# kubernetes-sigs/lws

Hardware: AMD Instinct MI355X
Metric: replica-group time-to-ready + rollout p50; Llama-3-70B 1-leader/0-worker TP=1 (lower is better)
Workload: dtype bf16; 1 GPU; model=llama-3-70b, global_batch=32, seq_len=128, parallelism=tp1, group=1-leader/0-workers (size=1), replicas=1, collectives_staged=False, orchestrator=lws_amd in-process control plane

## Files before the change

### lws_amd/cluster/statefulset_controller.py

```python
from __future__ import annotations

import re
from typing import Optional

from ..api import serde
from ..api.core import ControllerRevision, Pod, StatefulSet
from ..api.meta import OwnerReference, get_int_or_percent
from ..utils.hashutil import hash_object
from .controller import Controller, Manager
from .store import AlreadyExistsError, NotFoundError, Store

POD_NAME_RE = re.compile(r"^(.*)-([0-9]+)$")
STS_REVISION_LABEL = "controller-revision-hash"
STS_POD_NAME_LABEL = "statefulset.kubernetes.io/pod-name"
STS_OWNER_LABEL = "lws.amd.com/statefulset-name"


def parse_parent_and_ordinal(name: str) -> tuple[Optional[str], int]:
    m = POD_NAME_RE.match(name)
    if not m:
        return None, -1
    return m.group(1), int(m.group(2))


# ... 120 lines not shown
        cr = self.store.try_get("ControllerRevision", sts.metadata.namespace, name)
        if cr is None:
            return serde.deep_copy(sts.spec.template)
        from ..api.core import PodTemplateSpec
        return serde.from_dict(PodTemplateSpec, cr.data["template"])

    def _create_pod(self, sts: StatefulSet, ordinal: int, rev: str) -> None:
        template = self._template_for_revision(sts, rev)
        pod = Pod(metadata=serde.deep_copy(template.metadata),
                  spec=serde.deep_copy(template.spec))
        pod.metadata.name = f"{sts.metadata.name}-{ordinal}"
        pod.metadata.namespace = sts.metadata.namespace
        pod.metadata.labels = dict(template.metadata.labels or {})
        pod.metadata.labels[STS_REVISION_LABEL] = rev
        pod.metadata.labels[STS_POD_NAME_LABEL] = pod.metadata.name
        pod.metadata.labels[STS_OWNER_LABEL] = sts.metadata.name
        pod.metadata.annotations = dict(template.metadata.annotations or {})
        pod.metadata.owner_references = [OwnerReference(
            api_version=sts.api_version, kind=sts.kind, name=sts.metadata.name,
            uid=sts.metadata.uid, controller=True, block_owner_deletion=True)]
        pod.spec.hostname = pod.metadata.name
        if not pod.spec.subdomain:
            pod.spec.subdomain = sts.spec.service_name
        try:
            self.store.create(pod)
        except AlreadyExistsError:
            return
        self._ensure_pvcs(sts, pod)

    def _ensure_pvcs(self, sts: StatefulSet, pod: Pod) -> None:
        from ..api import serde as _serde

        created = self.store.try_get("Pod", pod.metadata.namespace,
                                     pod.metadata.name)
        if created is None:
            return
        policy = sts.spec.persistent_volume_claim_retention_policy
        for vct in sts.spec.volume_claim_templates or []:
            pvc = _serde.deep_copy(vct)
            pvc.metadata.name = f"{vct.metadata.name}-{pod.metadata.name}"
            pvc.metadata.namespace = sts.metadata.namespace
            pvc.metadata.labels = dict(vct.metadata.labels or {})
            pvc.metadata.labels[STS_OWNER_LABEL] = sts.metadata.name
            pvc.metadata.owner_references = []
            if policy is not None and policy.when_scaled == "Delete":
                pvc.metadata.owner_references = [OwnerReference(
# ... 54 lines not shown
```

### lws_amd/controllers/leaderworkerset_controller.py

```python
from __future__ import annotations

from typing import Optional

from ..api import leaderworkerset as lwsapi
from ..api import serde
from ..api.core import (RollingUpdateStatefulSetStrategy, Service,
                        ServiceSpec, StatefulSet, StatefulSetSpec,
                        StatefulSetUpdateStrategy)
from ..api.leaderworkerset import LeaderWorkerSet
from ..api.meta import (LabelSelector, OwnerReference, format_label_selector,
                        get_int_or_percent, new_condition)
from ..cluster.controller import Controller, Manager
from ..cluster.statefulset_controller import statefulset_ready
from ..cluster.store import AlreadyExistsError, Store
from ..utils import revision as revisionutils
from ..utils.podutils import pod_running_and_ready

FIELD_MANAGER = "lws"


def _merge_metadata(base: dict[str, str], overrides: dict[str, str]) -> dict[str, str]:
    out = dict(base or {})
    out.update(overrides)
    return out
# ... 333 lines not shown
             lwsapi.REVISION_KEY: revision_key})
        sts.metadata.annotations = _merge_metadata(
            lws.metadata.annotations,
            {lwsapi.REPLICAS_ANNOTATION_KEY: str(lws.spec.replicas)})
        sts.metadata.owner_references = [OwnerReference(
            api_version=lws.api_version, kind=lws.kind, name=lws.metadata.name,
            uid=lws.metadata.uid, controller=True, block_owner_deletion=True)]
        sts.spec = StatefulSetSpec(
            replicas=replicas,
            service_name=lws.metadata.name,
            pod_management_policy="Parallel",
            template=template,
            update_strategy=StatefulSetUpdateStrategy(
                type=lws.spec.rollout_strategy.type,
                rolling_update=RollingUpdateStatefulSetStrategy(
                    partition=partition,
                    max_unavailable=sts_max_unavailable)),
            selector=LabelSelector(match_labels={
                lwsapi.SET_NAME_LABEL_KEY: lws.metadata.name,
                lwsapi.WORKER_INDEX_LABEL_KEY: "0"}),
            volume_claim_templates=serde.deep_copy(t.volume_claim_templates),
            persistent_volume_claim_retention_policy=serde.deep_copy(
                t.persistent_volume_claim_retention_policy))
        self.store.apply(sts, field_manager=FIELD_MANAGER)

    def _reconcile_headless_services(self, lws) -> None:
        if lws.spec.network_config is not None and \
                lws.spec.network_config.subdomain_policy == \
                lwsapi.SubdomainPolicy.UniquePerReplica:
            return
        if self.store.try_get("Service", lws.metadata.namespace,
                              lws.metadata.name) is not None:
            return
        svc = Service()
        svc.metadata.name = lws.metadata.name
        svc.metadata.namespace = lws.metadata.namespace
        svc.spec = ServiceSpec(
            cluster_ip="None",
            selector={lwsapi.SET_NAME_LABEL_KEY: lws.metadata.name},
            publish_not_ready_addresses=True)
        svc.metadata.owner_references = [OwnerReference(
            api_version=lws.api_version, kind=lws.kind, name=lws.metadata.name,
            uid=lws.metadata.uid, controller=True, block_owner_deletion=True)]
        try:
            self.store.create(svc)
        except AlreadyExistsError:
# ... 101 lines not shown
```

### lws_amd/models/llama.py

```python
from __future__ import annotations

import math
from dataclasses import dataclass
import torch

from ..parallel.tp import ShardedLinear, all_gather_cat, all_reduce


@dataclass
class LlamaConfig:
    name: str = "llama"
    hidden_size: int = 4096
    intermediate_size: int = 14336
    num_layers: int = 32
    num_q_heads: int = 32
    num_kv_heads: int = 8
    head_dim: int = 128
    vocab_size: int = 128256
    rope_theta: float = 500000.0
    rms_eps: float = 1e-5
    max_position: int = 8192
    num_experts: int = 0
    num_experts_per_tok: int = 2

# ... 164 lines not shown
        else:
            lins += [self.gate_up, self.down]
        for lin in lins:
            lin.materialize(gen)
        self.input_norm.fill_(1.0)
        self.post_norm.fill_(1.0)

    @property
    def param_count(self) -> int:
        n = self.qkv.numel + self.o.numel
        n += self.input_norm.numel() + self.post_norm.numel()
        if self.router is not None:
            n += self.router.numel()
            n += sum(l.numel for l in self.experts_gate_up)
            n += sum(l.numel for l in self.experts_down)
        else:
            n += self.gate_up.numel + self.down.numel
        return n


class LlamaForCausalLM:
    def __init__(self, cfg: LlamaConfig, tp_rank: int = 0, tp_world: int = 1,
                 device: str = "cpu", dtype=torch.bfloat16,
                 pp_rank: int = 0, pp_world: int = 1):
        self.cfg = cfg
        self.tp_rank = tp_rank
        self.tp_world = tp_world
        self.pp_rank = pp_rank
        self.pp_world = pp_world
        assert tp_world == 1 or pp_world == 1, \
            "combined TP x PP grids are not supported"
        self.device = torch.device(device)
        self.dtype = dtype
        self._ops = _Ops(self.device)
        L, base, rem = cfg.num_layers, cfg.num_layers // pp_world, \
            cfg.num_layers % pp_world
        sizes = [base + (1 if r < rem else 0) for r in range(pp_world)]
        self.layer_offset = sum(sizes[:pp_rank])
        self.pp_first = pp_rank == 0
        self.pp_last = pp_rank == pp_world - 1
        self.layers = [LlamaLayer(cfg, tp_rank, tp_world, self.device, dtype)
                       for _ in range(sizes[pp_rank])]
        self.embed = torch.empty(cfg.vocab_size, cfg.hidden_size,
                                 device=self.device, dtype=dtype) \
            if self.pp_first else None
        self.final_norm = torch.empty(cfg.hidden_size, device=self.device,
                                      dtype=dtype) if self.pp_last else None
        self.lm_head = ShardedLinear(cfg.vocab_size, cfg.hidden_size, 0,
# ... 86 lines not shown
            k_cache[s // page, :, s % page] = k[t]
            v_cache[s // page, :, s % page] = v[t]

    def _qkv_views(self, qkv: torch.Tensor, layer, positions):
        d = self.cfg.head_dim
        if self._ops.is_gpu:
            q = qkv.narrow(-1, 0, layer.q_slice).unflatten(-1, (layer.hq, d))
            k = qkv.narrow(-1, layer.q_slice,
                           layer.kv_slice).unflatten(-1, (layer.hkv, d))
            v = qkv.narrow(-1, layer.q_slice + layer.kv_slice,
                           layer.kv_slice).unflatten(-1, (layer.hkv, d))
            self._ops.ops.rope(q, k, self.rope_table, positions,
                               layer.hq, layer.hkv)
            return q, k, v
        q, k, v = qkv.split([layer.q_slice, layer.kv_slice, layer.kv_slice],
                            dim=-1)
        q, k = self._ops.ref.rope_ref(q.contiguous(), k.contiguous(),
                                      self.rope_table, positions,
                                      layer.hq, layer.hkv)
        T = qkv.size(0)
        return (q.view(T, layer.hq, d), k.view(T, layer.hkv, d),
                v.contiguous().view(T, layer.hkv, d))

    def forward_prefill(self, batch: PrefillBatch, kv_caches) -> torch.Tensor:
        cfg = self.cfg
        if self.pp_first:
            x = self.embed[batch.input_ids]
            residual = None
        else:
            from ..parallel import pp as ppmod
            T = batch.input_ids.size(0)
            st = ppmod.recv_stage((2, T, cfg.hidden_size), self.dtype,
                                  self.device, self.pp_rank - 1)
            x, residual = st[0], st[1]
        for li, layer in enumerate(self.layers):
            if residual is None:
                residual = x
                h = self._rmsnorm(x, layer.input_norm)
            else:
                h, residual = self._fused_add_rmsnorm(x, residual,
                                                      layer.input_norm)
            qkv = layer.qkv(h)
            q, k, v = self._qkv_views(qkv, layer, batch.positions)
            k_cache, v_cache = kv_caches[li]
            self._write_cache(k, v, k_cache, v_cache, batch.slot_mapping)
            attn = self._prefill_attention(q, k, v, batch, layer,
                                           k_cache, v_cache)
# ... 33 lines not shown
        out = torch.empty(T, layer.hq * d, device=q.device, dtype=q.dtype)
        G = layer.hq // layer.hkv
        offs = q_offsets or [0] * (len(batch.seq_starts) - 1)
        for i in range(len(batch.seq_starts) - 1):
            s0, s1 = batch.seq_starts[i], batch.seq_starts[i + 1]
            kv0, kv1 = kv_starts[i], kv_starts[i + 1]
            S, KV, off = s1 - s0, kv1 - kv0, offs[i]
            qs = q[s0:s1].transpose(0, 1)
            ks = k[kv0:kv1].transpose(0, 1)
            vs = v[kv0:kv1].transpose(0, 1)
            ks = ks.repeat_interleave(G, dim=0)
            vs = vs.repeat_interleave(G, dim=0)
            scores = (qs @ ks.transpose(-1, -2)).float() * self.scale
            cols = torch.arange(KV, device=q.device)
            rows = torch.arange(S, device=q.device)
            mask = torch.where(cols[None, :] > off + rows[:, None],
                               float("-inf"), 0.0)
            p = torch.softmax(scores + mask, dim=-1).to(q.dtype)
            o = (p @ vs).transpose(0, 1).reshape(S, layer.hq * d)
            out[s0:s1] = o
        return out

    def forward_decode(self, batch: DecodeBatch, kv_caches) -> torch.Tensor:
        cfg = self.cfg
        if self.pp_first:
            x = self.embed[batch.input_ids]
            residual = None
        else:
            from ..parallel import pp as ppmod
            B0 = batch.input_ids.size(0)
            st = ppmod.recv_stage((2, B0, cfg.hidden_size), self.dtype,
                                  self.device, self.pp_rank - 1)
            x, residual = st[0], st[1]
        fp8q = (self._ops.is_gpu and self.layers
                and getattr(self.layers[0].qkv, "weight_fp8", None)
                is not None and self.layers[0].router is None
                and x.size(0) <= 32 and cfg.hidden_size % 256 == 0
                and self.layers[0].down.weight_fp8.size(1) % 256 == 0)
        for li, layer in enumerate(self.layers):
            if fp8q:
                if residual is None:
                    residual = x
                    h8, hs = self._ops.ops.rmsnorm_fp8(x, layer.input_norm,
                                                       cfg.rms_eps)
                else:
                    h8, hs = self._ops.ops.fused_add_rmsnorm_fp8(
# ... 113 lines not shown
```

### lws_amd/ops/__init__.py

```python
from __future__ import annotations

from pathlib import Path
from typing import Optional

import torch

_LIB = None
_LOAD_ERROR: Optional[str] = None


def _try_load() -> None:
    global _LIB, _LOAD_ERROR
    if _LIB is not None or _LOAD_ERROR is not None:
        return
    so = Path(__file__).resolve().parent / "_C.so"
    if not so.exists():
        _LOAD_ERROR = f"{so} not built (run python -m lws_amd.ops.build)"
        return
    try:
        torch.ops.load_library(str(so))
    except Exception:
        pass
    try:
        import importlib.util
# ... 53 lines not shown
    lib.rope(q, k, cos_sin, positions, num_q_heads, num_kv_heads)


def rope_and_cache(q, k, v, cos_sin, positions, k_cache, v_cache,
                   slot_mapping) -> None:
    lib = require_native()
    lib.rope_and_cache(q, k, v, cos_sin, positions, k_cache, v_cache,
                       slot_mapping)


def build_rope_table(max_pos: int, head_dim: int, theta: float = 10000.0,
                     device="cpu") -> torch.Tensor:
    half = head_dim // 2
    inv_freq = 1.0 / (theta ** (torch.arange(0, half, dtype=torch.float64) / half))
    pos = torch.arange(max_pos, dtype=torch.float64)
    ang = torch.outer(pos, inv_freq)
    table = torch.cat([torch.cos(ang), torch.sin(ang)], dim=-1).float()
    return table.to(device)


_PA_WS: dict = {}


def paged_attention_decode(q: torch.Tensor, k_cache: torch.Tensor,
                           v_cache: torch.Tensor, block_tables: torch.Tensor,
                           seq_lens: torch.Tensor, scale: float,
                           chunk_keys: Optional[int] = None,
                           workspace: Optional[tuple] = None,
                           out: Optional[torch.Tensor] = None) -> torch.Tensor:
    import os as _os

    lib = require_native()
    B, Hq, D = q.shape
    Hkv = k_cache.size(1)
    G = Hq // Hkv
    mfma = G in (4, 8, 16) and _os.environ.get("LWS_PA_MFMA", "1") != "0"
    max_len = int(block_tables.size(1)) * int(k_cache.size(2))
    if chunk_keys is None:
        if B * Hkv >= 256 and G == 1 and max_len <= 512:
            chunk_keys = ((max_len + 15) // 16) * 16
        else:
            if B * Hkv <= 64:
                if mfma:
                    target_chunks = max(1, min(8, -(-max_len // 64)))
                else:
                    target_chunks = min(16, (max_len + 31) // 32)
            else:
                target_chunks = max(1, min(4, -(-max_len // 96)))
            chunk_keys = -(-max_len // target_chunks)
            chunk_keys = ((chunk_keys + 15) // 16) * 16
    num_chunks = max(1, (max_len + chunk_keys - 1) // chunk_keys)
    if mfma:
        num_chunks *= 4
    if workspace is None:
        key = ("paws", B, Hkv, num_chunks, G, q.device.index)
        ws = _PA_WS.get(key)
        if ws is None:
            ws = (torch.empty((B, Hkv, num_chunks, G, D),
                              dtype=torch.float32, device=q.device),
                  torch.empty((B, Hkv, num_chunks, G, 2),
                              dtype=torch.float32, device=q.device))
            _PA_WS[key] = ws
        ws_acc, ws_ml = ws
    else:
        ws_acc, ws_ml = workspace
        num_chunks = ws_ml.size(2)
    if out is None:
        out = torch.empty_like(q)
    lib.paged_attention_decode(out, q, k_cache, v_cache, block_tables,
                               seq_lens, ws_acc, ws_ml, scale, chunk_keys)
    return out


def reshape_and_cache(k: torch.Tensor, v: torch.Tensor, k_cache: torch.Tensor,
                      v_cache: torch.Tensor, slot_mapping: torch.Tensor) -> None:
    lib = require_native()
    lib.reshape_and_cache(k, v, k_cache, v_cache, slot_mapping)


SKINNY_GEMM_MAX_M = 32
_SKINNY_WS: dict = {}


def skinny_gemm(x: torch.Tensor, w: torch.Tensor,
                out: Optional[torch.Tensor] = None) -> torch.Tensor:
    lib = require_native()
    grouped = x.dim() == 3
    E = x.size(0) if grouped else 1
    M, K = x.shape[-2], x.shape[-1]
    N = w.size(-2)
    if out is None:
        shape = (E, M, N) if grouped else (M, N)
        out = torch.empty(shape, dtype=x.dtype, device=x.device)
    import os
    target = int(os.environ.get("LWS_SG_TARGET", "256"))
    n_blocks = (N + 63) // 64
    split = min(max(1, target // max(1, n_blocks)), max(1, K // 128))
    k_slice = (K // split + 127) // 128 * 128
    grid_y = (K + k_slice - 1) // k_slice
    if grouped and E * n_blocks >= 256:
        grid_y = 1
    key = (grid_y, E, M, N, x.device.index)
    ws = _SKINNY_WS.get(key)
    if ws is None:
        ws = torch.empty(grid_y, E * M, N, dtype=torch.float32,
                         device=x.device)
        _SKINNY_WS[key] = ws
    lib.skinny_gemm(out, x, w, ws)
    return out


_SKINNY_FP8_BUFS: dict = {}


def skinny_gemm_fp8(x: torch.Tensor, w8: torch.Tensor, w_scale: torch.Tensor,
                    out: Optional[torch.Tensor] = None) -> torch.Tensor:
    lib = require_native()
    M, K = x.shape
    N = w8.size(0)
    if out is None:
        out = torch.empty(M, N, dtype=torch.bfloat16, device=x.device)
    import os
    target = int(os.environ.get("LWS_SG8_TARGET", "512"))
    ksub = int(os.environ.get("LWS_SG8_KSUB", "128"))
    rows = 32 if (os.environ.get("LWS_SG8_ROWS") == "32"
                  and ksub == 128) else 64
    n_blocks = (N + rows - 1) // rows
    split = min(max(1, target // max(1, n_blocks)), max(1, K // ksub))
    k_slice = (K // split + ksub - 1) // ksub * ksub
    grid_y = (K + k_slice - 1) // k_slice
    key = (grid_y, M, N, K, x.device.index)
    bufs = _SKINNY_FP8_BUFS.get(key)
# ... 87 lines not shown
    rows, D = x.shape[0], x.shape[-1]
    y8, ys = _fp8_act_buffers(rows, D, x.device)
    lib.fused_add_rmsnorm_fp8(y8, ys, x.contiguous(), residual, weight, eps)
    return y8, ys


def silu_mul_fp8(gateup: torch.Tensor) -> tuple:
    lib = require_native()
    rows = gateup.shape[0]
    I = gateup.shape[-1] // 2
    a8, ascale = _fp8_act_buffers(rows, I, gateup.device)
    lib.silu_mul_fp8(a8, ascale, gateup.contiguous())
    return a8, ascale


def prefill_attention(q: torch.Tensor, k: torch.Tensor, v: torch.Tensor,
                      seq_starts: list, scale: float,
                      out: Optional[torch.Tensor] = None,
                      kv_starts: Optional[list] = None,
                      q_offsets: Optional[list] = None) -> torch.Tensor:
    lib = require_native()
    T, Hq, D = q.shape
    device = q.device
    B = len(seq_starts) - 1
    tile_seq, tile_q0 = [], []
    for i in range(B):
        S = seq_starts[i + 1] - seq_starts[i]
        for q0 in range(0, S, 64):
            tile_seq.append(i)
            tile_q0.append(q0)
    if kv_starts is None:
        kv_starts = seq_starts
    if q_offsets is None:
        q_offsets = [0] * B
    if out is None:
        out = torch.empty(T, Hq * D, dtype=q.dtype, device=device)
    lib.prefill_attention(
        out, q, k, v,
        torch.tensor(tile_seq, dtype=torch.int32, device=device),
        torch.tensor(tile_q0, dtype=torch.int32, device=device),
        torch.tensor(seq_starts, dtype=torch.int32, device=device),
        torch.tensor(kv_starts, dtype=torch.int32, device=device),
        torch.tensor(q_offsets, dtype=torch.int32, device=device), scale)
    return out
```

### lws_amd/ops/build.py

```python
from __future__ import annotations

import os
import shutil
import sys
from pathlib import Path

PKG_DIR = Path(__file__).resolve().parent
CSRC = PKG_DIR / "csrc"
SO_NAME = "_C.so"
SOURCES = ["norm_act.hip", "rope.hip", "paged_attention.hip",
           "skinny_gemm.hip", "skinny_gemm_fp8.hip", "prefill_attention.hip",
           "bindings.cpp"]


def _newest_source_mtime() -> float:
    return max((CSRC / s).stat().st_mtime for s in SOURCES) if CSRC.exists() else 0


def needs_build() -> bool:
    so = PKG_DIR / SO_NAME
    if not so.exists():
        return True
    return so.stat().st_mtime < _newest_source_mtime()


def build(verbose: bool = False, force: bool = False) -> Path:
    so_path = PKG_DIR / SO_NAME
    if not force and not needs_build():
        return so_path

    os.environ.setdefault("PYTORCH_ROCM_ARCH", "gfx950")
    from torch.utils.cpp_extension import load

    build_dir = PKG_DIR / "build"
    build_dir.mkdir(exist_ok=True)
# ... 21 lines not shown
```

### lws_amd/ops/csrc/bindings.cpp

```cpp
#include <torch/extension.h>

void rmsnorm(torch::Tensor out, torch::Tensor input, torch::Tensor weight,
             double eps);
void fused_add_rmsnorm(torch::Tensor x, torch::Tensor residual,
                       torch::Tensor weight, double eps);
void silu_mul(torch::Tensor out, torch::Tensor gateup);
void rmsnorm_fp8(torch::Tensor out8, torch::Tensor oscale,
                 torch::Tensor input, torch::Tensor weight, double eps);
void fused_add_rmsnorm_fp8(torch::Tensor out8, torch::Tensor oscale,
                           torch::Tensor x, torch::Tensor residual,
                           torch::Tensor weight, double eps);
void silu_mul_fp8(torch::Tensor out8, torch::Tensor oscale,
                  torch::Tensor gateup);
void rope(torch::Tensor q, torch::Tensor k, torch::Tensor cos_sin,
          torch::Tensor positions, long long num_q_heads,
          long long num_kv_heads);
void rope_and_cache(torch::Tensor q, torch::Tensor k, torch::Tensor v,
                    torch::Tensor cos_sin, torch::Tensor positions,
                    torch::Tensor k_cache, torch::Tensor v_cache,
                    torch::Tensor slot_mapping);
void paged_attention_decode(torch::Tensor out, torch::Tensor q,
                            torch::Tensor k_cache, torch::Tensor v_cache,
                            torch::Tensor block_tables, torch::Tensor seq_lens,
                            torch::Tensor ws_acc, torch::Tensor ws_ml,
                            double scale, long long chunk_keys);
void reshape_and_cache(torch::Tensor k, torch::Tensor v,
                       torch::Tensor k_cache, torch::Tensor v_cache,
                       torch::Tensor slot_mapping);
void skinny_gemm(torch::Tensor out, torch::Tensor x, torch::Tensor w,
                 torch::Tensor ws);
void skinny_gemm_fp8(torch::Tensor out, torch::Tensor x8, torch::Tensor xs,
                     torch::Tensor w8, torch::Tensor ws_n, torch::Tensor ws);
void quant_fp8_rows(torch::Tensor x8, torch::Tensor xs, torch::Tensor x);
void prefill_attention(torch::Tensor out, torch::Tensor q, torch::Tensor k,
                       torch::Tensor v, torch::Tensor tile_seq,
                       torch::Tensor tile_q0, torch::Tensor seq_starts,
                       torch::Tensor kv_starts, torch::Tensor q_offs,
                       double scale);

PYBIND11_MODULE(TORCH_EXTENSION_NAME, m) {
  m.def("rmsnorm", &rmsnorm, "RMSNorm (bf16, gfx950)");
  m.def("fused_add_rmsnorm", &fused_add_rmsnorm,
        "in-place residual add + RMSNorm (bf16, gfx950)");
  m.def("silu_mul", &silu_mul, "fused SiLU-gate multiply (bf16, gfx950)");
  m.def("rmsnorm_fp8", &rmsnorm_fp8,
        "RMSNorm with fused per-token e4m3 quantization epilogue");
  m.def("fused_add_rmsnorm_fp8", &fused_add_rmsnorm_fp8,
        "residual add + RMSNorm with fused e4m3 quantization epilogue");
  m.def("silu_mul_fp8", &silu_mul_fp8,
        "SiLU-gate multiply with fused e4m3 quantization epilogue");
  m.def("rope", &rope, "fused rotary embedding for q,k (bf16, gfx950)");
  m.def("rope_and_cache", &rope_and_cache,
        "rope on q in place + rotated k and v scattered into the paged "
        "KV cache (single decode launch)");
  m.def("paged_attention_decode", &paged_attention_decode,
        "GQA paged attention decode with flash-decoding chunk split");
  m.def("reshape_and_cache", &reshape_and_cache,
        "scatter new k/v into the paged KV cache");
  m.def("skinny_gemm", &skinny_gemm,
        "split-K MFMA GEMM for decode-shape projections (M<=32)");
  m.def("skinny_gemm_fp8", &skinny_gemm_fp8,
        "W8A8 e4m3 split-K MFMA GEMM for decode projections (M<=32)");
  m.def("quant_fp8_rows", &quant_fp8_rows,
// ... 5 lines not shown
```

### lws_amd/parallel/tp.py

```python
from __future__ import annotations

import os
from dataclasses import dataclass
from typing import Optional

import torch
import torch.distributed as dist


@dataclass
class ParallelState:
    rank: int = 0
    world_size: int = 1
    local_rank: int = 0
    device: torch.device = torch.device("cpu")
    group: Optional[object] = None
    staged: bool = False

    @property
    def is_distributed(self) -> bool:
        return self.world_size > 1


_STATE = ParallelState()
# ... 92 lines not shown

    def __call__(self, x: torch.Tensor) -> torch.Tensor:
        if self.weight_fp8 is not None:
            M = x.size(0)
            if not x.is_cuda:
                wf = self.weight_fp8.float() * self.scale_fp8[:, None]
                return (x.float() @ wf.t()).to(torch.bfloat16)
            if x.dim() == 2 and M <= 32 and x.size(1) % 256 == 0:
                from .. import ops
                return ops.skinny_gemm_fp8(x, self.weight_fp8,
                                           self.scale_fp8)
            pad = (-M) % 16
            if pad:
                x = torch.nn.functional.pad(x, (0, 0, 0, pad))
            xs = (x.abs().amax().float() / 448.0).clamp(min=1e-8)
            x8 = (x.float() / xs).clamp(-448.0, 448.0).to(torch.float8_e4m3fn)
            if self._ones is None or self._ones.device != x.device:
                self._ones = torch.ones((), device=x.device)
            out = torch._scaled_mm(x8, self.weight_fp8.t(), scale_a=xs,
                                   scale_b=self._ones,
                                   out_dtype=torch.bfloat16)
            out = out * self.scale_fp8.to(torch.bfloat16)[None, :]
            return out[:M] if pad else out
        if x.is_cuda and x.dim() == 2 and x.size(0) <= 32 and \
                x.size(1) % 128 == 0 and self._skinny_wins():
            from .. import ops
            return ops.skinny_gemm(x.contiguous(), self.weight)
        return x @ self.weight.t()

    def _skinny_wins(self) -> bool:
        N, K = self.weight.shape
        if N * K <= 32 * 1024 * 1024:
            return True
        if K <= 4096:
            return True
        if K >= 16384 and N >= 8192:
            return True
        return False

    def forward_q8(self, x8: torch.Tensor, xs: torch.Tensor) -> torch.Tensor:
        from .. import ops
        return ops.skinny_gemm_fp8_q(x8, xs, self.weight_fp8, self.scale_fp8)

    @property
    def numel(self) -> int:
        w = self.weight if self.weight is not None else self.weight_fp8
        return w.numel()
```

### lws_amd/serving/engine.py

```python
from __future__ import annotations

import time
from dataclasses import dataclass, field
from typing import Optional

import torch

from ..models.llama import (DecodeBatch, LlamaConfig, LlamaForCausalLM,
                            MODEL_PRESETS, PrefillBatch)

PAGE_SIZE = 16


@dataclass
class EngineConfig:
    model: str = "llama-tiny"
    kv_pages: int = 256
    max_batch: int = 64
    max_model_len: int = 2048
    max_prefill_tokens: int = 8192
    weight_dtype: str = "bf16"
    seed: int = 0
    device: str = "cpu"
    tp_rank: int = 0
    tp_world: int = 1
    pp_rank: int = 0
    pp_world: int = 1


@dataclass
class SamplingParams:

    temperature: float = 0.0
    top_p: float = 1.0
    top_k: int = 0
    seed: Optional[int] = None
    stop_token: Optional[int] = None

    @property
    def greedy(self) -> bool:
        return self.temperature <= 0.0


@dataclass
class Sequence:
    seq_id: int
    token_ids: list[int]
    pages: list[int] = field(default_factory=list)
    num_cached: int = 0
    finished: bool = False
# ... 11 lines not shown

    def alloc(self, n: int) -> list[int]:
        if n > len(self.free):
            raise RuntimeError("KV cache exhausted")
        return [self.free.pop() for _ in range(n)]

    def release(self, pages: list[int]) -> None:
        self.free.extend(pages)


class Engine:
    def __init__(self, cfg: EngineConfig,
                 model_cfg: Optional[LlamaConfig] = None):
        self.cfg = cfg
        mc = model_cfg or MODEL_PRESETS[cfg.model]()
        self.model_cfg = mc
        if cfg.max_model_len <= 0:
            cfg.max_model_len = mc.max_position
        cfg.max_model_len = min(cfg.max_model_len, mc.max_position)
        self.model = LlamaForCausalLM(mc, tp_rank=cfg.tp_rank,
                                      tp_world=cfg.tp_world,
                                      device=cfg.device,
                                      pp_rank=cfg.pp_rank,
                                      pp_world=cfg.pp_world)
        self.device = self.model.device
        self.kv_caches: list[tuple[torch.Tensor, torch.Tensor]] = []
        self.allocator = BlockAllocator(cfg.kv_pages)
        self.sequences: dict[int, Sequence] = {}
        self._next_seq_id = 0
        self.ready = False
        import os
        self._graphs: dict[tuple[int, int], "_CapturedDecode"] = {}
        graphs_ok = ((cfg.tp_world == 1 and cfg.pp_world == 1)
                     or os.environ.get("LWS_AMD_GRAPHS", "0") == "1")
        self.use_graphs = (self.device.type == "cuda" and graphs_ok
                           and os.environ.get("LWS_AMD_NO_GRAPHS", "0") != "1")

    def _load_gemm_tuning(self) -> None:
        from pathlib import Path
        csv = Path(__file__).resolve().parent.parent / "ops" / \
            "tunableop_gemm.csv"
        if not csv.exists():
            return
        try:
            import torch.cuda.tunable as tunable
            tunable.enable(True)
            tunable.tuning_enable(False)
            tunable.read_file(str(csv))
        except Exception:
            pass

    def load(self) -> dict:
        t0 = time.perf_counter()
        if self.device.type == "cuda":
            self._load_gemm_tuning()
        n_params = self.model.materialize(self.cfg.seed)
        if self.cfg.weight_dtype == "fp8":
            assert self.device.type == "cuda", "fp8 mode is GPU-only"
            self.model.quantize_fp8()
            torch.cuda.empty_cache()
        if self.device.type == "cuda":
            torch.cuda.synchronize()
        t1 = time.perf_counter()
        nl, hkv = self.model.kv_cache_spec()
        d = self.model_cfg.head_dim
        self.kv_caches = []
        for _ in range(nl):
            k = torch.zeros(self.cfg.kv_pages, hkv, PAGE_SIZE, d,
                            device=self.device, dtype=torch.bfloat16)
            v = torch.zeros_like(k)
            self.kv_caches.append((k, v))
        if self.device.type == "cuda":
            torch.cuda.synchronize()
        t2 = time.perf_counter()
        self._warmup()
        if self.device.type == "cuda":
            torch.cuda.synchronize()
        t3 = time.perf_counter()
        self.ready = True
        return {"params": n_params, "weights_s": t1 - t0, "kv_s": t2 - t1,
                "warmup_s": t3 - t2,
                "warmup_detail": getattr(self, "warmup_detail", None)}

    def _warmup(self) -> None:
        sid = self.add_request([1, 2, 3, 4])
        graphs = self.use_graphs
        self.use_graphs = False
        try:
            t0 = time.perf_counter()
            self.step()
            if self.device.type == "cuda":
                torch.cuda.synchronize()
            t1 = time.perf_counter()
            self.step()
# ... 361 lines not shown
```

Baseline: 303.3 ms.

## Run transformer layer loop natively in C++ and batch KV/tile allocations

Adds a C++ layer loop (forward_layers_prefill/decode) that runs all attention and MLP blocks in one native call instead of per-layer Python dispatch. It also packs prefill tile metadata into a single host-to-device tensor, allocates all KV caches as one slab, and factors out the workspace planning helpers. Separately, the controllers now check the live owner object before creating pods or applying StatefulSets. The main aim is to cut Python launch overhead during warmup and serving, at the cost of a new native build dependency and extra store lookups in the controllers.

```diff
diff --git a/lws_amd/cluster/statefulset_controller.py b/lws_amd/cluster/statefulset_controller.py
--- a/lws_amd/cluster/statefulset_controller.py
+++ b/lws_amd/cluster/statefulset_controller.py
@@ -166,6 +166,11 @@
         pod.spec.hostname = pod.metadata.name
         if not pod.spec.subdomain:
             pod.spec.subdomain = sts.spec.service_name
+        live = self.store.try_get("StatefulSet", sts.metadata.namespace,
+                                  sts.metadata.name)
+        if live is None or live.metadata.uid != sts.metadata.uid or \
+                live.metadata.deletion_timestamp is not None:
+            return
         try:
             self.store.create(pod)
         except AlreadyExistsError:
diff --git a/lws_amd/controllers/leaderworkerset_controller.py b/lws_amd/controllers/leaderworkerset_controller.py
--- a/lws_amd/controllers/leaderworkerset_controller.py
+++ b/lws_amd/controllers/leaderworkerset_controller.py
@@ -379,6 +379,11 @@
             volume_claim_templates=serde.deep_copy(t.volume_claim_templates),
             persistent_volume_claim_retention_policy=serde.deep_copy(
                 t.persistent_volume_claim_retention_policy))
+        live = self.store.try_get(lwsapi.KIND, lws.metadata.namespace,
+                                  lws.metadata.name)
+        if live is None or live.metadata.uid != lws.metadata.uid or \
+                live.metadata.deletion_timestamp is not None:
+            return
         self.store.apply(sts, field_manager=FIELD_MANAGER)
 
     def _reconcile_headless_services(self, lws) -> None:
diff --git a/lws_amd/models/llama.py b/lws_amd/models/llama.py
--- a/lws_amd/models/llama.py
+++ b/lws_amd/models/llama.py
@@ -210,8 +210,10 @@
 class LlamaForCausalLM:
     def __init__(self, cfg: LlamaConfig, tp_rank: int = 0, tp_world: int = 1,
                  device: str = "cpu", dtype=torch.bfloat16,
-                 pp_rank: int = 0, pp_world: int = 1):
+                 pp_rank: int = 0, pp_world: int = 1,
+                 native_layers: bool = True):
         self.cfg = cfg
+        self.native_layers = native_layers
         self.tp_rank = tp_rank
         self.tp_world = tp_world
         self.pp_rank = pp_rank
@@ -344,7 +346,112 @@
         return (q.view(T, layer.hq, d), k.view(T, layer.hkv, d),
                 v.contiguous().view(T, layer.hkv, d))
 
+    def _native_ok(self) -> bool:
+        return (self.native_layers and self._ops.is_gpu
+                and self.pp_world == 1 and bool(self.layers)
+                and self.layers[0].router is None
+                and self.layers[0].qkv.weight_fp8 is None)
+
+    def _native_plan(self, M: int) -> tuple:
+        ops = self._ops.ops
+        L = self.layers
+        weights = ([l.input_norm for l in L], [l.qkv.weight for l in L],
+                   [l.o.weight for l in L], [l.post_norm for l in L],
+                   [l.gate_up.weight for l in L], [l.down.weight for l in L])
+        lins = (L[0].qkv, L[0].o, L[0].gate_up, L[0].down)
+        skinny = [int(lin.use_skinny(M)) for lin in lins]
+        if getattr(self, "_no_ws", None) is None:
+            self._no_ws = torch.empty(0, dtype=torch.float32,
+                                      device=self.device)
+        ws = [ops.skinny_workspace(M, lin.weight.size(0), lin.weight.size(1),
+                                   self.device) if use else self._no_ws
+              for lin, use in zip(lins, skinny)]
+        return weights, skinny, ws
+
+    def _forward_prefill_native(self, batch: PrefillBatch,
+                                kv_caches) -> torch.Tensor:
+        cfg = self.cfg
+        ops = self._ops.ops
+        lib = ops.require_native()
+        x = self.embed[batch.input_ids]
+        l0 = self.layers[0]
+        weights, skinny, ws = self._native_plan(x.size(0))
+        chunked = batch.kv_row_idx is not None
+        tiles = list(ops.prefill_tiles(
+            batch.seq_starts, self.device,
+            batch.kv_starts if chunked else None,
+            batch.q_offsets if chunked else None))
+        if self.tp_world == 1:
+            out = lib.forward_layers_prefill(
+                x, *weights, [k for k, _ in kv_caches],
+                [v for _, v in kv_caches], self.rope_table, batch.positions,
+                batch.slot_mapping, tiles, batch.kv_row_idx, skinny, ws,
+                l0.hq, l0.hkv, cfg.rms_eps, self.scale)
+        else:
+            bufs = lib.alloc_layer_buffers(
+                x, l0.qkv.weight.size(0), l0.o.weight.size(1),
+                l0.gate_up.weight.size(0))
+            for li, layer in enumerate(self.layers):
+                k_cache, v_cache = kv_caches[li]
+                lib.attn_block_prefill(
+                    bufs, x, li == 0, layer.input_norm, layer.qkv.weight,
+                    layer.o.weight, k_cache, v_cache, self.rope_table,
+                    batch.positions, batch.slot_mapping, tiles,
+                    batch.kv_row_idx, skinny, ws, l0.hq, l0.hkv,
+                    cfg.rms_eps, self.scale)
+                self._ar(bufs[4])
+                lib.mlp_block(bufs, x, layer.post_norm, layer.gate_up.weight,
+                              layer.down.weight, skinny, ws, l0.hq, l0.hkv,
+                              cfg.rms_eps)
+                self._ar(bufs[5])
+            out = bufs[5]
+        h, _ = self._fused_add_rmsnorm(out, x, self.final_norm)
+        last = torch.tensor([s - 1 for s in batch.seq_starts[1:]],
+                            device=h.device, dtype=torch.long)
+        return h[last]
+
+    def _forward_decode_native(self, batch: DecodeBatch,
+                               kv_caches) -> torch.Tensor:
+        cfg = self.cfg
+        ops = self._ops.ops
+        lib = ops.require_native()
+        x = self.embed[batch.input_ids]
+        l0 = self.layers[0]
+        weights, skinny, ws = self._native_plan(x.size(0))
+        chunk_keys, ws_acc, ws_ml = ops.paged_attention_plan(
+            x.size(0), l0.hq, cfg.head_dim, kv_caches[0][0],
+            batch.block_tables)
+        if self.tp_world == 1:
+            out = lib.forward_layers_decode(
+                x, *weights, [k for k, _ in kv_caches],
+                [v for _, v in kv_caches], self.rope_table, batch.positions,
+                batch.slot_mapping, batch.block_tables, batch.seq_lens,
+                ws_acc, ws_ml, chunk_keys, skinny, ws, l0.hq, l0.hkv,
+                cfg.rms_eps, self.scale)
+        else:
+            bufs = lib.alloc_layer_buffers(
+                x, l0.qkv.weight.size(0), l0.o.weight.size(1),
+                l0.gate_up.weight.size(0))
+            for li, layer in enumerate(self.layers):
+                k_cache, v_cache = kv_caches[li]
+                lib.attn_block_decode(
+                    bufs, x, li == 0, layer.input_norm, layer.qkv.weight,
+                    layer.o.weight, k_cache, v_cache, self.rope_table,
+                    batch.positions, batch.slot_mapping, batch.block_tables,
+                    batch.seq_lens, ws_acc, ws_ml, chunk_keys, skinny, ws,
+                    l0.hq, l0.hkv, cfg.rms_eps, self.scale)
+                self._ar(bufs[4])
+                lib.mlp_block(bufs, x, layer.post_norm, layer.gate_up.weight,
+                              layer.down.weight, skinny, ws, l0.hq, l0.hkv,
+                              cfg.rms_eps)
+                self._ar(bufs[5])
+            out = bufs[5]
+        h, _ = self._fused_add_rmsnorm(out, x, self.final_norm)
+        return h
+
     def forward_prefill(self, batch: PrefillBatch, kv_caches) -> torch.Tensor:
+        if self._native_ok():
+            return self._forward_prefill_native(batch, kv_caches)
         cfg = self.cfg
         if self.pp_first:
             x = self.embed[batch.input_ids]
@@ -424,6 +531,8 @@
         return out
 
     def forward_decode(self, batch: DecodeBatch, kv_caches) -> torch.Tensor:
+        if self._native_ok():
+            return self._forward_decode_native(batch, kv_caches)
         cfg = self.cfg
         if self.pp_first:
             x = self.embed[batch.input_ids]
diff --git a/lws_amd/ops/__init__.py b/lws_amd/ops/__init__.py
--- a/lws_amd/ops/__init__.py
+++ b/lws_amd/ops/__init__.py
@@ -99,16 +99,12 @@
 _PA_WS: dict = {}
 
 
-def paged_attention_decode(q: torch.Tensor, k_cache: torch.Tensor,
-                           v_cache: torch.Tensor, block_tables: torch.Tensor,
-                           seq_lens: torch.Tensor, scale: float,
-                           chunk_keys: Optional[int] = None,
-                           workspace: Optional[tuple] = None,
-                           out: Optional[torch.Tensor] = None) -> torch.Tensor:
+def paged_attention_plan(B: int, Hq: int, D: int, k_cache: torch.Tensor,
+                         block_tables: torch.Tensor,
+                         chunk_keys: Optional[int] = None,
+                         workspace: Optional[tuple] = None) -> tuple:
     import os as _os
 
-    lib = require_native()
-    B, Hq, D = q.shape
     Hkv = k_cache.size(1)
     G = Hq // Hkv
     mfma = G in (4, 8, 16) and _os.environ.get("LWS_PA_MFMA", "1") != "0"
@@ -126,22 +122,33 @@
                 target_chunks = max(1, min(4, -(-max_len // 96)))
             chunk_keys = -(-max_len // target_chunks)
             chunk_keys = ((chunk_keys + 15) // 16) * 16
+    if workspace is not None:
+        return chunk_keys, workspace[0], workspace[1]
     num_chunks = max(1, (max_len + chunk_keys - 1) // chunk_keys)
     if mfma:
         num_chunks *= 4
-    if workspace is None:
-        key = ("paws", B, Hkv, num_chunks, G, q.device.index)
-        ws = _PA_WS.get(key)
-        if ws is None:
-            ws = (torch.empty((B, Hkv, num_chunks, G, D),
-                              dtype=torch.float32, device=q.device),
-                  torch.empty((B, Hkv, num_chunks, G, 2),
-                              dtype=torch.float32, device=q.device))
-            _PA_WS[key] = ws
-        ws_acc, ws_ml = ws
-    else:
-        ws_acc, ws_ml = workspace
-        num_chunks = ws_ml.size(2)
+    device = k_cache.device
+    key = ("paws", B, Hkv, num_chunks, G, device.index)
+    ws = _PA_WS.get(key)
+    if ws is None:
+        ws = (torch.empty((B, Hkv, num_chunks, G, D),
+                          dtype=torch.float32, device=device),
+              torch.empty((B, Hkv, num_chunks, G, 2),
+                          dtype=torch.float32, device=device))
+        _PA_WS[key] = ws
+    return chunk_keys, ws[0], ws[1]
+
+
+def paged_attention_decode(q: torch.Tensor, k_cache: torch.Tensor,
+                           v_cache: torch.Tensor, block_tables: torch.Tensor,
+                           seq_lens: torch.Tensor, scale: float,
+                           chunk_keys: Optional[int] = None,
+                           workspace: Optional[tuple] = None,
+                           out: Optional[torch.Tensor] = None) -> torch.Tensor:
+    lib = require_native()
+    B, Hq, D = q.shape
+    chunk_keys, ws_acc, ws_ml = paged_attention_plan(
+        B, Hq, D, k_cache, block_tables, chunk_keys, workspace)
     if out is None:
         out = torch.empty_like(q)
     lib.paged_attention_decode(out, q, k_cache, v_cache, block_tables,
@@ -169,7 +176,15 @@
     if out is None:
         shape = (E, M, N) if grouped else (M, N)
         out = torch.empty(shape, dtype=x.dtype, device=x.device)
+    ws = skinny_workspace(M, N, K, x.device, E=E, grouped=grouped)
+    lib.skinny_gemm(out, x, w, ws)
+    return out
+
+
+def skinny_workspace(M: int, N: int, K: int, device, E: int = 1,
+                     grouped: bool = False) -> torch.Tensor:
     import os
+    device = torch.device(device)
     target = int(os.environ.get("LWS_SG_TARGET", "256"))
     n_blocks = (N + 63) // 64
     split = min(max(1, target // max(1, n_blocks)), max(1, K // 128))
@@ -177,14 +192,13 @@
     grid_y = (K + k_slice - 1) // k_slice
     if grouped and E * n_blocks >= 256:
         grid_y = 1
-    key = (grid_y, E, M, N, x.device.index)
+    key = (grid_y, E, M, N, device.index)
     ws = _SKINNY_WS.get(key)
     if ws is None:
         ws = torch.empty(grid_y, E * M, N, dtype=torch.float32,
-                         device=x.device)
+                         device=device)
         _SKINNY_WS[key] = ws
-    lib.skinny_gemm(out, x, w, ws)
-    return out
+    return ws
 
 
 _SKINNY_FP8_BUFS: dict = {}
@@ -318,6 +332,17 @@
     lib = require_native()
     T, Hq, D = q.shape
     device = q.device
+    if out is None:
+        out = torch.empty(T, Hq * D, dtype=q.dtype, device=device)
+    lib.prefill_attention(
+        out, q, k, v,
+        *prefill_tiles(seq_starts, device, kv_starts, q_offsets), scale)
+    return out
+
+
+def prefill_tiles(seq_starts: list, device,
+                  kv_starts: Optional[list] = None,
+                  q_offsets: Optional[list] = None) -> tuple:
     B = len(seq_starts) - 1
     tile_seq, tile_q0 = [], []
     for i in range(B):
@@ -329,13 +354,7 @@
         kv_starts = seq_starts
     if q_offsets is None:
         q_offsets = [0] * B
-    if out is None:
-        out = torch.empty(T, Hq * D, dtype=q.dtype, device=device)
-    lib.prefill_attention(
-        out, q, k, v,
-        torch.tensor(tile_seq, dtype=torch.int32, device=device),
-        torch.tensor(tile_q0, dtype=torch.int32, device=device),
-        torch.tensor(seq_starts, dtype=torch.int32, device=device),
-        torch.tensor(kv_starts, dtype=torch.int32, device=device),
-        torch.tensor(q_offsets, dtype=torch.int32, device=device), scale)
-    return out
+    parts = (tile_seq, tile_q0, seq_starts, kv_starts, q_offsets)
+    flat = torch.tensor([v for p in parts for v in p], dtype=torch.int32,
+                        device=device)
+    return flat.split([len(p) for p in parts])
diff --git a/lws_amd/ops/build.py b/lws_amd/ops/build.py
--- a/lws_amd/ops/build.py
+++ b/lws_amd/ops/build.py
@@ -10,7 +10,7 @@
 SO_NAME = "_C.so"
 SOURCES = ["norm_act.hip", "rope.hip", "paged_attention.hip",
            "skinny_gemm.hip", "skinny_gemm_fp8.hip", "prefill_attention.hip",
-           "bindings.cpp"]
+           "layer_loop.cpp", "bindings.cpp"]
 
 
 def _newest_source_mtime() -> float:
diff --git a/lws_amd/ops/csrc/bindings.cpp b/lws_amd/ops/csrc/bindings.cpp
--- a/lws_amd/ops/csrc/bindings.cpp
+++ b/lws_amd/ops/csrc/bindings.cpp
@@ -38,7 +38,75 @@
                        torch::Tensor kv_starts, torch::Tensor q_offs,
                        double scale);
 
+std::vector<torch::Tensor> alloc_layer_buffers(torch::Tensor x,
+                                               long long qkv_n,
+                                               long long attn_n,
+                                               long long gate_up_n);
+void attn_block_prefill(std::vector<torch::Tensor> bufs,
+                        torch::Tensor residual, bool first,
+                        torch::Tensor norm_w, torch::Tensor w_qkv,
+                        torch::Tensor w_o, torch::Tensor k_cache,
+                        torch::Tensor v_cache, torch::Tensor rope_table,
+                        torch::Tensor positions, torch::Tensor slot_mapping,
+                        std::vector<torch::Tensor> tiles,
+                        c10::optional<torch::Tensor> kv_row_idx,
+                        std::vector<int64_t> use_skinny,
+                        std::vector<torch::Tensor> skinny_ws, long long hq,
+                        long long hkv, double eps, double scale);
+void attn_block_decode(std::vector<torch::Tensor> bufs,
+                       torch::Tensor residual, bool first,
+                       torch::Tensor norm_w, torch::Tensor w_qkv,
+                       torch::Tensor w_o, torch::Tensor k_cache,
+                       torch::Tensor v_cache, torch::Tensor rope_table,
+                       torch::Tensor positions, torch::Tensor slot_mapping,
+                       torch::Tensor block_tables, torch::Tensor seq_lens,
+                       torch::Tensor ws_acc, torch::Tensor ws_ml,
+                       long long chunk_keys, std::vector<int64_t> use_skinny,
+                       std::vector<torch::Tensor> skinny_ws, long long hq,
+                       long long hkv, double eps, double scale);
+void mlp_block(std::vector<torch::Tensor> bufs, torch::Tensor residual,
+               torch::Tensor norm_w, torch::Tensor w_gate_up,
+               torch::Tensor w_down, std::vector<int64_t> use_skinny,
+               std::vector<torch::Tensor> skinny_ws, long long hq,
+               long long hkv, double eps);
+torch::Tensor forward_layers_prefill(
+    torch::Tensor x, std::vector<torch::Tensor> input_norms,
+    std::vector<torch::Tensor> w_qkv, std::vector<torch::Tensor> w_o,
+    std::vector<torch::Tensor> post_norms,
+    std::vector<torch::Tensor> w_gate_up, std::vector<torch::Tensor> w_down,
+    std::vector<torch::Tensor> k_caches, std::vector<torch::Tensor> v_caches,
+    torch::Tensor rope_table, torch::Tensor positions,
+    torch::Tensor slot_mapping, std::vector<torch::Tensor> tiles,
+    c10::optional<torch::Tensor> kv_row_idx, std::vector<int64_t> use_skinny,
+    std::vector<torch::Tensor> skinny_ws, long long hq, long long hkv,
+    double eps, double scale);
+torch::Tensor forward_layers_decode(
+    torch::Tensor x, std::vector<torch::Tensor> input_norms,
+    std::vector<torch::Tensor> w_qkv, std::vector<torch::Tensor> w_o,
+    std::vector<torch::Tensor> post_norms,
+    std::vector<torch::Tensor> w_gate_up, std::vector<torch::Tensor> w_down,
+    std::vector<torch::Tensor> k_caches, std::vector<torch::Tensor> v_caches,
+    torch::Tensor rope_table, torch::Tensor positions,
+    torch::Tensor slot_mapping, torch::Tensor block_tables,
+    torch::Tensor seq_lens, torch::Tensor ws_acc, torch::Tensor ws_ml,
+    long long chunk_keys, std::vector<int64_t> use_skinny,
+    std::vector<torch::Tensor> skinny_ws, long long hq, long long hkv,
+    double eps, double scale);
+
 PYBIND11_MODULE(TORCH_EXTENSION_NAME, m) {
+  using nogil = py::call_guard<py::gil_scoped_release>;
+  m.def("alloc_layer_buffers", &alloc_layer_buffers, nogil(),
+        "activation buffers shared by every layer of one forward");
+  m.def("attn_block_prefill", &attn_block_prefill, nogil(),
+        "one layer, input norm .. o-projection, prefill");
+  m.def("attn_block_decode", &attn_block_decode, nogil(),
+        "one layer, input norm .. o-projection, paged decode");
+  m.def("mlp_block", &mlp_block, nogil(),
+        "one layer, post norm .. down-projection");
+  m.def("forward_layers_prefill", &forward_layers_prefill, nogil(),
+        "all dense bf16 layers of a prefill forward (tp_world == 1)");
+  m.def("forward_layers_decode", &forward_layers_decode, nogil(),
+        "all dense bf16 layers of a decode forward (tp_world == 1)");
   m.def("rmsnorm", &rmsnorm, "RMSNorm (bf16, gfx950)");
   m.def("fused_add_rmsnorm", &fused_add_rmsnorm,
         "in-place residual add + RMSNorm (bf16, gfx950)");
diff --git a/lws_amd/ops/csrc/layer_loop.cpp b/lws_amd/ops/csrc/layer_loop.cpp
--- /dev/null
+++ b/lws_amd/ops/csrc/layer_loop.cpp
@@ -0,0 +1,285 @@
+#include <torch/extension.h>
+
+#include <vector>
+
+void rmsnorm(torch::Tensor out, torch::Tensor input, torch::Tensor weight,
+             double eps);
+void fused_add_rmsnorm(torch::Tensor x, torch::Tensor residual,
+                       torch::Tensor weight, double eps);
+void silu_mul(torch::Tensor out, torch::Tensor gateup);
+void rope(torch::Tensor q, torch::Tensor k, torch::Tensor cos_sin,
+          torch::Tensor positions, long long num_q_heads,
+          long long num_kv_heads);
+void rope_and_cache(torch::Tensor q, torch::Tensor k, torch::Tensor v,
+                    torch::Tensor cos_sin, torch::Tensor positions,
+                    torch::Tensor k_cache, torch::Tensor v_cache,
+                    torch::Tensor slot_mapping);
+void paged_attention_decode(torch::Tensor out, torch::Tensor q,
+                            torch::Tensor k_cache, torch::Tensor v_cache,
+                            torch::Tensor block_tables, torch::Tensor seq_lens,
+                            torch::Tensor ws_acc, torch::Tensor ws_ml,
+                            double scale, long long chunk_keys);
+void reshape_and_cache(torch::Tensor k, torch::Tensor v,
+                       torch::Tensor k_cache, torch::Tensor v_cache,
+                       torch::Tensor slot_mapping);
+void skinny_gemm(torch::Tensor out, torch::Tensor x, torch::Tensor w,
+                 torch::Tensor ws);
+void prefill_attention(torch::Tensor out, torch::Tensor q, torch::Tensor k,
+                       torch::Tensor v, torch::Tensor tile_seq,
+                       torch::Tensor tile_q0, torch::Tensor seq_starts,
+                       torch::Tensor kv_starts, torch::Tensor q_offs,
+                       double scale);
+
+namespace {
+
+using torch::Tensor;
+using TensorList = std::vector<Tensor>;
+
+constexpr long long HEAD_DIM = 128;
+enum { P_QKV = 0, P_O = 1, P_GATE_UP = 2, P_DOWN = 3, P_COUNT = 4 };
+enum { T_SEQ = 0, T_Q0 = 1, T_SEQ_STARTS = 2, T_KV_STARTS = 3, T_Q_OFFS = 4,
+       T_COUNT = 5 };
+
+struct GemmPlan {
+  std::vector<int64_t> skinny;
+  TensorList ws;
+};
+
+struct Buffers {
+  Tensor qkv, attn, gate_up, act, xo, xd;
+  Tensor q, k, v;
+};
+
+Buffers make_buffers(const TensorList& b, long long hq, long long hkv) {
+  TORCH_CHECK(b.size() == 6, "layer buffers: expected 6 tensors");
+  Buffers s{b[0], b[1], b[2], b[3], b[4], b[5], {}, {}, {}};
+  const long long qs = hq * HEAD_DIM, kvs = hkv * HEAD_DIM;
+  TORCH_CHECK(s.qkv.dim() == 2 && s.qkv.size(1) == qs + 2 * kvs,
+              "qkv buffer does not match the head counts");
+  s.q = s.qkv.narrow(-1, 0, qs).unflatten(-1, {hq, HEAD_DIM});
+  s.k = s.qkv.narrow(-1, qs, kvs).unflatten(-1, {hkv, HEAD_DIM});
+  s.v = s.qkv.narrow(-1, qs + kvs, kvs).unflatten(-1, {hkv, HEAD_DIM});
+  return s;
+}
+
+TensorList alloc_buffers(const Tensor& x, long long qkv_n, long long attn_n,
+                         long long gate_up_n) {
+  const long long T = x.size(0), H = x.size(1);
+  auto opt = x.options();
+  return {at::empty({T, qkv_n}, opt),       at::empty({T, attn_n}, opt),
+          at::empty({T, gate_up_n}, opt),   at::empty({T, gate_up_n / 2}, opt),
+          at::empty({T, H}, opt),           at::empty({T, H}, opt)};
+}
+
+void check_plan(const GemmPlan& p) {
+  TORCH_CHECK(p.skinny.size() == P_COUNT && p.ws.size() == P_COUNT,
+              "gemm plan: expected one flag and one workspace per projection");
+}
+
+void linear(Tensor& out, const Tensor& x, const Tensor& w,
+            const GemmPlan& plan, int slot) {
+  if (plan.skinny[slot])
+    skinny_gemm(out, x, w, plan.ws[slot]);
+  else
+    at::mm_out(out, x, w.t());
+}
+
+void input_norm(Buffers& b, const Tensor& residual, bool first,
+                const Tensor& weight, double eps) {
+  if (first)
+    rmsnorm(b.xd, residual, weight, eps);
+  else
+    fused_add_rmsnorm(b.xd, residual, weight, eps);
+}
+
+
+void attn_prefill(Buffers& b, const Tensor& residual, bool first,
+                  const Tensor& norm_w, const Tensor& w_qkv,
+                  const Tensor& w_o, const Tensor& k_cache,
+                  const Tensor& v_cache, const Tensor& rope_table,
+                  const Tensor& positions, const Tensor& slot_mapping,
+                  const TensorList& tiles,
+                  const c10::optional<Tensor>& kv_row_idx,
+                  const GemmPlan& plan, long long hq, long long hkv,
+                  double eps, double scale) {
+  input_norm(b, residual, first, norm_w, eps);
+  linear(b.qkv, b.xd, w_qkv, plan, P_QKV);
+  rope(b.q, b.k, rope_table, positions, hq, hkv);
+  reshape_and_cache(b.k, b.v, k_cache, v_cache, slot_mapping);
+  Tensor k = b.k, v = b.v;
+  if (kv_row_idx.has_value()) {
+    k = at::index_select(k_cache.reshape({-1, HEAD_DIM}), 0, *kv_row_idx)
+            .view({-1, hkv, HEAD_DIM});
+    v = at::index_select(v_cache.reshape({-1, HEAD_DIM}), 0, *kv_row_idx)
+            .view({-1, hkv, HEAD_DIM});
+  }
+  prefill_attention(b.attn, b.q, k, v, tiles[T_SEQ], tiles[T_Q0],
+                    tiles[T_SEQ_STARTS], tiles[T_KV_STARTS], tiles[T_Q_OFFS],
+                    scale);
+  linear(b.xo, b.attn, w_o, plan, P_O);
+}
+
+void attn_decode(Buffers& b, const Tensor& residual, bool first,
+                 const Tensor& norm_w, const Tensor& w_qkv, const Tensor& w_o,
+                 const Tensor& k_cache, const Tensor& v_cache,
+                 const Tensor& rope_table, const Tensor& positions,
+                 const Tensor& slot_mapping, const Tensor& block_tables,
+                 const Tensor& seq_lens, const Tensor& ws_acc,
+                 const Tensor& ws_ml, long long chunk_keys,
+                 const GemmPlan& plan, long long hq, double eps,
+                 double scale) {
+  input_norm(b, residual, first, norm_w, eps);
+  linear(b.qkv, b.xd, w_qkv, plan, P_QKV);
+  rope_and_cache(b.q, b.k, b.v, rope_table, positions, k_cache, v_cache,
+                 slot_mapping);
+  paged_attention_decode(b.attn.view({-1, hq, HEAD_DIM}), b.q, k_cache,
+                         v_cache, block_tables, seq_lens, ws_acc, ws_ml,
+                         scale, chunk_keys);
+  linear(b.xo, b.attn, w_o, plan, P_O);
+}
+
+
+void mlp(Buffers& b, const Tensor& residual, const Tensor& norm_w,
+         const Tensor& w_gate_up, const Tensor& w_down, const GemmPlan& plan,
+         double eps) {
+  fused_add_rmsnorm(b.xo, residual, norm_w, eps);
+  linear(b.gate_up, b.xo, w_gate_up, plan, P_GATE_UP);
+  silu_mul(b.act, b.gate_up);
+  linear(b.xd, b.act, w_down, plan, P_DOWN);
+}
+
+void check_layers(size_t n, const TensorList& a, const char* what) {
+  TORCH_CHECK(a.size() == n, "layer loop: ", what, " has ", a.size(),
+              " entries for ", n, " layers");
+}
+
+}
+
+
+std::vector<torch::Tensor> alloc_layer_buffers(torch::Tensor x,
+                                               long long qkv_n,
+                                               long long attn_n,
+                                               long long gate_up_n) {
+  return alloc_buffers(x, qkv_n, attn_n, gate_up_n);
+}
+
+void attn_block_prefill(std::vector<torch::Tensor> bufs,
+                        torch::Tensor residual, bool first,
+                        torch::Tensor norm_w, torch::Tensor w_qkv,
+                        torch::Tensor w_o, torch::Tensor k_cache,
+                        torch::Tensor v_cache, torch::Tensor rope_table,
+                        torch::Tensor positions, torch::Tensor slot_mapping,
+                        std::vector<torch::Tensor> tiles,
+                        c10::optional<torch::Tensor> kv_row_idx,
+                        std::vector<int64_t> use_skinny,
+                        std::vector<torch::Tensor> skinny_ws, long long hq,
+                        long long hkv, double eps, double scale) {
+  GemmPlan plan{use_skinny, skinny_ws};
+  check_plan(plan);
+  TORCH_CHECK(tiles.size() == T_COUNT, "prefill tiles: expected 5 tensors");
+  Buffers b = make_buffers(bufs, hq, hkv);
+  attn_prefill(b, residual, first, norm_w, w_qkv, w_o, k_cache, v_cache,
+               rope_table, positions, slot_mapping, tiles, kv_row_idx, plan,
+               hq, hkv, eps, scale);
+}
+
+void attn_block_decode(std::vector<torch::Tensor> bufs,
+                       torch::Tensor residual, bool first,
+                       torch::Tensor norm_w, torch::Tensor w_qkv,
+                       torch::Tensor w_o, torch::Tensor k_cache,
+                       torch::Tensor v_cache, torch::Tensor rope_table,
+                       torch::Tensor positions, torch::Tensor slot_mapping,
+                       torch::Tensor block_tables, torch::Tensor seq_lens,
+                       torch::Tensor ws_acc, torch::Tensor ws_ml,
+                       long long chunk_keys, std::vector<int64_t> use_skinny,
+                       std::vector<torch::Tensor> skinny_ws, long long hq,
+                       long long hkv, double eps, double scale) {
+  GemmPlan plan{use_skinny, skinny_ws};
+  check_plan(plan);
+  Buffers b = make_buffers(bufs, hq, hkv);
+  attn_decode(b, residual, first, norm_w, w_qkv, w_o, k_cache, v_cache,
+              rope_table, positions, slot_mapping, block_tables, seq_lens,
+              ws_acc, ws_ml, chunk_keys, plan, hq, eps, scale);
+}
+
+void mlp_block(std::vector<torch::Tensor> bufs, torch::Tensor residual,
+               torch::Tensor norm_w, torch::Tensor w_gate_up,
+               torch::Tensor w_down, std::vector<int64_t> use_skinny,
+               std::vector<torch::Tensor> skinny_ws, long long hq,
+               long long hkv, double eps) {
+  GemmPlan plan{use_skinny, skinny_ws};
+  check_plan(plan);
+  Buffers b = make_buffers(bufs, hq, hkv);
+  mlp(b, residual, norm_w, w_gate_up, w_down, plan, eps);
+}
+
+torch::Tensor forward_layers_prefill(
+    torch::Tensor x, std::vector<torch::Tensor> input_norms,
+    std::vector<torch::Tensor> w_qkv, std::vector<torch::Tensor> w_o,
+    std::vector<torch::Tensor> post_norms,
+    std::vector<torch::Tensor> w_gate_up, std::vector<torch::Tensor> w_down,
+    std::vector<torch::Tensor> k_caches, std::vector<torch::Tensor> v_caches,
+    torch::Tensor rope_table, torch::Tensor positions,
+    torch::Tensor slot_mapping, std::vector<torch::Tensor> tiles,
+    c10::optional<torch::Tensor> kv_row_idx, std::vector<int64_t> use_skinny,
+    std::vector<torch::Tensor> skinny_ws, long long hq, long long hkv,
+    double eps, double scale) {
+  const size_t L = w_qkv.size();
+  TORCH_CHECK(L > 0, "layer loop: no layers");
+  check_layers(L, input_norms, "input_norms");
+  check_layers(L, w_o, "w_o");
+  check_layers(L, post_norms, "post_norms");
+  check_layers(L, w_gate_up, "w_gate_up");
+  check_layers(L, w_down, "w_down");
+  check_layers(L, k_caches, "k_caches");
+  check_layers(L, v_caches, "v_caches");
+  GemmPlan plan{use_skinny, skinny_ws};
+  check_plan(plan);
+  TORCH_CHECK(tiles.size() == T_COUNT, "prefill tiles: expected 5 tensors");
+  Buffers b = make_buffers(
+      alloc_buffers(x, w_qkv[0].size(0), w_o[0].size(1),
+                    w_gate_up[0].size(0)), hq, hkv);
+  for (size_t l = 0; l < L; ++l) {
+    attn_prefill(b, x, l == 0, input_norms[l], w_qkv[l], w_o[l], k_caches[l],
+                 v_caches[l], rope_table, positions, slot_mapping, tiles,
+                 kv_row_idx, plan, hq, hkv, eps, scale);
+    mlp(b, x, post_norms[l], w_gate_up[l], w_down[l], plan, eps);
+  }
+  return b.xd;
+}
+
+torch::Tensor forward_layers_decode(
+    torch::Tensor x, std::vector<torch::Tensor> input_norms,
+    std::vector<torch::Tensor> w_qkv, std::vector<torch::Tensor> w_o,
+    std::vector<torch::Tensor> post_norms,
+    std::vector<torch::Tensor> w_gate_up, std::vector<torch::Tensor> w_down,
+    std::vector<torch::Tensor> k_caches, std::vector<torch::Tensor> v_caches,
+    torch::Tensor rope_table, torch::Tensor positions,
+    torch::Tensor slot_mapping, torch::Tensor block_tables,
+    torch::Tensor seq_lens, torch::Tensor ws_acc, torch::Tensor ws_ml,
+    long long chunk_keys, std::vector<int64_t> use_skinny,
+    std::vector<torch::Tensor> skinny_ws, long long hq, long long hkv,
+    double eps, double scale) {
+  const size_t L = w_qkv.size();
+  TORCH_CHECK(L > 0, "layer loop: no layers");
+  check_layers(L, input_norms, "input_norms");
+  check_layers(L, w_o, "w_o");
+  check_layers(L, post_norms, "post_norms");
+  check_layers(L, w_gate_up, "w_gate_up");
+  check_layers(L, w_down, "w_down");
+  check_layers(L, k_caches, "k_caches");
+  check_layers(L, v_caches, "v_caches");
+  GemmPlan plan{use_skinny, skinny_ws};
+  check_plan(plan);
+  Buffers b = make_buffers(
+      alloc_buffers(x, w_qkv[0].size(0), w_o[0].size(1),
+                    w_gate_up[0].size(0)), hq, hkv);
+  for (size_t l = 0; l < L; ++l) {
+    attn_decode(b, x, l == 0, input_norms[l], w_qkv[l], w_o[l], k_caches[l],
+                v_caches[l], rope_table, positions, slot_mapping,
+                block_tables, seq_lens, ws_acc, ws_ml, chunk_keys, plan, hq,
+                eps, scale);
+    mlp(b, x, post_norms[l], w_gate_up[l], w_down[l], plan, eps);
+  }
+  return b.xd;
+}
diff --git a/lws_amd/parallel/tp.py b/lws_amd/parallel/tp.py
--- a/lws_amd/parallel/tp.py
+++ b/lws_amd/parallel/tp.py
@@ -138,11 +138,14 @@
                                    out_dtype=torch.bfloat16)
             out = out * self.scale_fp8.to(torch.bfloat16)[None, :]
             return out[:M] if pad else out
-        if x.is_cuda and x.dim() == 2 and x.size(0) <= 32 and \
-                x.size(1) % 128 == 0 and self._skinny_wins():
+        if x.is_cuda and x.dim() == 2 and self.use_skinny(x.size(0)):
             from .. import ops
             return ops.skinny_gemm(x.contiguous(), self.weight)
         return x @ self.weight.t()
+
+    def use_skinny(self, M: int) -> bool:
+        return M <= 32 and self.weight.size(1) % 128 == 0 \
+            and self._skinny_wins()
 
     def _skinny_wins(self) -> bool:
         N, K = self.weight.shape
diff --git a/lws_amd/serving/engine.py b/lws_amd/serving/engine.py
--- a/lws_amd/serving/engine.py
+++ b/lws_amd/serving/engine.py
@@ -26,6 +26,7 @@
     tp_world: int = 1
     pp_rank: int = 0
     pp_world: int = 1
+    native_layers: bool = True
 
 
 @dataclass
@@ -83,7 +84,8 @@
                                       tp_world=cfg.tp_world,
                                       device=cfg.device,
                                       pp_rank=cfg.pp_rank,
-                                      pp_world=cfg.pp_world)
+                                      pp_world=cfg.pp_world,
+                                      native_layers=cfg.native_layers)
         self.device = self.model.device
         self.kv_caches: list[tuple[torch.Tensor, torch.Tensor]] = []
         self.allocator = BlockAllocator(cfg.kv_pages)
@@ -125,12 +127,9 @@
         t1 = time.perf_counter()
         nl, hkv = self.model.kv_cache_spec()
         d = self.model_cfg.head_dim
-        self.kv_caches = []
-        for _ in range(nl):
-            k = torch.zeros(self.cfg.kv_pages, hkv, PAGE_SIZE, d,
-                            device=self.device, dtype=torch.bfloat16)
-            v = torch.zeros_like(k)
-            self.kv_caches.append((k, v))
+        slab = torch.zeros(2 * nl, self.cfg.kv_pages, hkv, PAGE_SIZE, d,
+                           device=self.device, dtype=torch.bfloat16)
+        self.kv_caches = [(slab[2 * i], slab[2 * i + 1]) for i in range(nl)]
         if self.device.type == "cuda":
             torch.cuda.synchronize()
         t2 = time.perf_counter()
```

Measured after the change: 189.7 ms (median of 6 runs). 37.5% less time.
